# LessUp/n-body

Hardware: AMD Instinct MI355X
Metric: pair_interactions_per_s (higher is better)
Workload: dtype f32; 1 GPU; plummer_N1048576_direct_n2_velocity_verlet; bodies=1048576, seed=42, deterministic=True, deterministic_mode=1

## Files before the change

### n-body_amd/csrc/direct_sym.hip

```cpp

#include <type_traits>

#include "common.h"

namespace nbh {

typedef float f2 __attribute__((ext_vector_type(2)));

__device__ __forceinline__ float wave_rot1(float v) {
  return __int_as_float(__builtin_amdgcn_mov_dpp(__float_as_int(v), 0x134 , 0xF, 0xF, false));
}

constexpr int kSymBlocksPerCU = 16;
constexpr int kSymMinChunks = 4;
constexpr float kFar = 1.0e18f;

template <int R, bool RECT, bool EQM, bool DET = false>
__global__ __launch_bounds__(kBlock) void direct_sym_kernel(const float4* __restrict__ posm, int n,
                                                            const float4* __restrict__ posj, int nj,
                                                            int NB, int NBJ, int chunks_per_split,
                                                            double* __restrict__ acc64,
                                                            void* __restrict__ accj,
                                                            size_t plane_i, size_t plane_j,
                                                            const unsigned int* __restrict__ mass_range,
                                                            float eps2) {
  const bool uniform = mass_range[0] == mass_range[1] && mass_range[2] == mass_range[3] &&
                       mass_range[0] == mass_range[2] && ordered_to_float(mass_range[0]) > 0.f;
  if (uniform != EQM) return;
  const float m0 = EQM ? ordered_to_float(mass_range[0]) : 1.0f;
  constexpr int S = kBlock * R;
  __shared__ float slab[2][4][3][64];
  const int tid = threadIdx.x, lane = tid & 63, w = tid >> 6;
  const int A = blockIdx.x;
  const int D = RECT ? NBJ - 1 : NB / 2;
  constexpr int CPB = kBlock * R / 64;
  const int q0 = blockIdx.y * chunks_per_split;
  const int q1 = min((D + 1) * CPB, q0 + chunks_per_split);
  if (q0 >= q1) {
    if constexpr (DET) {
#pragma unroll
      for (int r = 0; r < R; r++)
#pragma unroll
        for (int c = 0; c < 3; c++)
          acc64[((size_t)blockIdx.y * 3 + c) * plane_i + (size_t)(A * S + r * kBlock + tid)] = 0.0;
    }
    return;
  }

  f2 xi[R / 2], yi[R / 2], zi[R / 2], mi[R / 2];
#pragma unroll
  for (int r = 0; r < R / 2; r++) {
    float4 p0 = make_float4(kFar, kFar, kFar, 0.f), p1 = p0;
    const int i0 = A * S + (2 * r) * kBlock + tid, i1 = i0 + kBlock;
    if (i0 < n) p0 = posm[i0];
    if (i1 < n) p1 = posm[i1];
    xi[r] = f2{p0.x, p1.x}; yi[r] = f2{p0.y, p1.y}; zi[r] = f2{p0.z, p1.z}; mi[r] = f2{p0.w, p1.w};
  }
  constexpr bool LACC = R >= 8;
  constexpr int RR = LACC ? 1 : R;
  __shared__ double lacc[LACC ? 3 * R * kBlock : 1];
  double sx[RR], sy[RR], sz[RR];
  if constexpr (LACC) {
#pragma unroll
    for (int k = 0; k < 3 * R; k++) lacc[k * kBlock + tid] = 0.0;
  } else {
#pragma unroll
    for (int r = 0; r < R; r++) sx[r] = sy[r] = sz[r] = 0.0;
  }
  f2 ax[R / 2], ay[R / 2], az[R / 2];
#pragma unroll
  for (int r = 0; r < R / 2; r++) ax[r] = ay[r] = az[r] = f2{0.f, 0.f};
  const f2 e2 = {eps2, eps2};

  auto partner_valid = [&](int d) { return RECT || !((NB % 2 == 0) && d == D && d > 0 && A >= D); };
  const int nchunks = q1 - q0;

  auto load_chunk = [&](int q) -> float4 {
    const int d = (q0 + q) / CPB, c = (q0 + q) % CPB;
    const int B = RECT ? d : (A + d) % NB;
    const int j = B * S + c * 64 + lane;
    float4 p = make_float4(kFar, kFar, kFar, 0.f);
    if (RECT) { if (j < nj) p = posj[j]; }
    else if (j < n && partner_valid(d)) p = posm[j];
    return p;
  };
  auto flush_chunk = [&](int q) {
    const int pd = (q0 + q) / CPB, pc = (q0 + q) % CPB;
    if constexpr (DET) {
      if (RECT || pd > 0) {
        const size_t plane = RECT ? plane_j : plane_i;
        float* slot = static_cast<float*>(accj) + (size_t)(RECT ? A : pd - 1) * 3 * plane;
        const unsigned int j = (unsigned int)((RECT ? pd : (A + pd) % NB) * S + pc * 64 + lane), pl = (unsigned int)plane;
        const int sb = q & 1;
        const bool keep = partner_valid(pd);
#pragma unroll
        for (int c = 0; c < 3; c++) {
          const float v = (slab[sb][0][c][lane] + slab[sb][1][c][lane]) + (slab[sb][2][c][lane] + slab[sb][3][c][lane]);
          slot[c * pl + j] = keep ? v : 0.f;
        }
      }
    } else if ((RECT || pd > 0) && partner_valid(pd)) {
      const int j = (RECT ? pd : (A + pd) % NB) * S + pc * 64 + lane;
      const int sb = q & 1;
      double* dst = RECT ? static_cast<double*>(accj) : acc64;
      const size_t plane = RECT ? plane_j : plane_i;
#pragma unroll
      for (int c = 0; c < 3; c++) {
        const float v = (slab[sb][0][c][lane] + slab[sb][1][c][lane]) + (slab[sb][2][c][lane] + slab[sb][3][c][lane]);
        unsafeAtomicAdd(&dst[c * plane + (size_t)j], (double)v * (double)m0);
      }
    }
  };

  float4 jnext = load_chunk(0);
  for (int q = 0; q < nchunks; q++) {
    const float4 jcur = jnext;
    if (q + 1 < nchunks) jnext = load_chunk(q + 1);
    const int d = (q0 + q) / CPB;
    const bool react = RECT || d > 0;
    if (q > 0) {
      __syncthreads();
      if (w == (q & 3)) flush_chunk(q - 1);
    }
    float jx = jcur.x, jy = jcur.y, jz = jcur.z, jm = jcur.w;
    float hjx = 0.f, hjy = 0.f, hjz = 0.f;
    auto steps = [&](auto react_tag) {
      constexpr bool REACT = decltype(react_tag)::value;
      constexpr int kStepUnroll = R >= 16 ? 1 : 2;
#pragma unroll kStepUnroll
      for (int k = 0; k < 64; k++) {
        const f2 sxj = {jx, jx}, syj = {jy, jy}, szj = {jz, jz}, smj = {jm, jm};
        f2 dx[R / 2], dy[R / 2], dz[R / 2], g[R / 2];
#pragma unroll
        for (int r = 0; r < R / 2; r++) {
          dx[r] = sxj - xi[r]; dy[r] = syj - yi[r]; dz[r] = szj - zi[r];
          g[r] = __builtin_elementwise_fma(dx[r], dx[r], __builtin_elementwise_fma(dy[r], dy[r], __builtin_elementwise_fma(dz[r], dz[r], e2)));
        }
#pragma unroll
        for (int r = 0; r < R / 2; r++) {
          g[r].x = __builtin_amdgcn_rsqf(g[r].x);
          g[r].y = __builtin_amdgcn_rsqf(g[r].y);
        }
#pragma unroll
        for (int r = 0; r < R / 2; r++) g[r] = (g[r] * g[r]) * g[r];
        f2 hx = {hjx, 0.f}, hy = {hjy, 0.f}, hz = {hjz, 0.f};
#pragma unroll
        for (int r = 0; r < R / 2; r++) {
          const f2 fj = EQM ? g[r] : g[r] * smj;
          ax[r] = __builtin_elementwise_fma(fj, dx[r], ax[r]);
          ay[r] = __builtin_elementwise_fma(fj, dy[r], ay[r]);
          az[r] = __builtin_elementwise_fma(fj, dz[r], az[r]);
          if (REACT) {
            const f2 fi = EQM ? g[r] : g[r] * mi[r];
            hx = __builtin_elementwise_fma(-fi, dx[r], hx);
            hy = __builtin_elementwise_fma(-fi, dy[r], hy);
            hz = __builtin_elementwise_fma(-fi, dz[r], hz);
          }
        }
        if (REACT) {
          hjx = wave_rot1(hx.x + hx.y); hjy = wave_rot1(hy.x + hy.y); hjz = wave_rot1(hz.x + hz.y);
        }
        jx = wave_rot1(jx); jy = wave_rot1(jy); jz = wave_rot1(jz); jm = wave_rot1(jm);
      }
    };
    if constexpr (R >= 12 && !EQM) {
      (void)react;
      steps(std::true_type{});
    } else {
      if (react) steps(std::true_type{}); else steps(std::false_type{});
    }
    slab[q & 1][w][0][lane] = hjx; slab[q & 1][w][1][lane] = hjy; slab[q & 1][w][2][lane] = hjz;
    if ((q & 3) == 3 || q == nchunks - 1) {
#pragma unroll
      for (int r = 0; r < R / 2; r++) {
        if constexpr (LACC) {
          lacc[(0 * R + 2 * r) * kBlock + tid] += (double)ax[r].x; lacc[(0 * R + 2 * r + 1) * kBlock + tid] += (double)ax[r].y;
          lacc[(1 * R + 2 * r) * kBlock + tid] += (double)ay[r].x; lacc[(1 * R + 2 * r + 1) * kBlock + tid] += (double)ay[r].y;
          lacc[(2 * R + 2 * r) * kBlock + tid] += (double)az[r].x; lacc[(2 * R + 2 * r + 1) * kBlock + tid] += (double)az[r].y;
        } else {
          sx[2 * r] += (double)ax[r].x; sx[2 * r + 1] += (double)ax[r].y;
          sy[2 * r] += (double)ay[r].x; sy[2 * r + 1] += (double)ay[r].y;
          sz[2 * r] += (double)az[r].x; sz[2 * r + 1] += (double)az[r].y;
        }
        ax[r] = ay[r] = az[r] = f2{0.f, 0.f};
      }
    }
  }
  __syncthreads();
  if (w == (nchunks & 3)) flush_chunk(nchunks - 1);
#pragma unroll
  for (int r = 0; r < R; r++) {
    const int i = A * S + r * kBlock + tid;
    const double fx = LACC ? lacc[(0 * R + r) * kBlock + tid] : sx[LACC ? 0 : r];
    const double fy = LACC ? lacc[(1 * R + r) * kBlock + tid] : sy[LACC ? 0 : r];
    const double fz = LACC ? lacc[(2 * R + r) * kBlock + tid] : sz[LACC ? 0 : r];
    if constexpr (DET) {
      double* slot = acc64 + (size_t)blockIdx.y * 3 * plane_i;
      const unsigned int iu = (unsigned int)i, pl = (unsigned int)plane_i;
      slot[iu] = fx;
      slot[pl + iu] = fy;
      slot[2u * pl + iu] = fz;
    } else {
      unsafeAtomicAdd(&acc64[(size_t)i], fx * (double)m0);
      unsafeAtomicAdd(&acc64[plane_i + (size_t)i], fy * (double)m0);
      unsafeAtomicAdd(&acc64[2 * plane_i + (size_t)i], fz * (double)m0);
    }
  }
}

__global__ void mass_range_init_kernel(unsigned int* enc) {
  if (threadIdx.x < 4) enc[threadIdx.x] = (threadIdx.x & 1) ? 0u : 0xffffffffu;
}

__global__ __launch_bounds__(kBlock) void mass_range_kernel(const float4* __restrict__ posm, int n,
                                                            unsigned int* __restrict__ enc) {
  __shared__ float red[4][2];
  float lo = INFINITY, hi = -INFINITY;
  for (int i = blockIdx.x * kBlock + threadIdx.x; i < n; i += gridDim.x * kBlock) {
    const float m = posm[i].w;
    lo = fminf(lo, m); hi = fmaxf(hi, m);
  }
#pragma unroll
  for (int off = 32; off > 0; off >>= 1) {
    lo = fminf(lo, __shfl_down(lo, off, 64));
    hi = fmaxf(hi, __shfl_down(hi, off, 64));
  }
  const int w = threadIdx.x >> 6;
  if ((threadIdx.x & 63) == 0) { red[w][0] = lo; red[w][1] = hi; }
  __syncthreads();
  if (threadIdx.x == 0) {
    for (int k = 1; k < 4; k++) { lo = fminf(lo, red[k][0]); hi = fmaxf(hi, red[k][1]); }
    atomicMin(&enc[0], float_to_ordered(fminf(lo, red[0][0])));
    atomicMax(&enc[1], float_to_ordered(fmaxf(hi, red[0][1])));
  }
}

struct SlotLayout {
  const double* isl;
  const float* rsl;
  size_t plane;
  int n_i, n_r;
};

__global__ __launch_bounds__(kBlock) void direct_sym_finalize_kernel(
    SlotLayout eq, SlotLayout gen, int apply_m0, const unsigned int* __restrict__ mass_range, int n, float G,
    float4* __restrict__ acc4, int accumulate, float* __restrict__ ax, float* __restrict__ ay, float* __restrict__ az,
    float* __restrict__ vx, float* __restrict__ vy, float* __restrict__ vz, const float* __restrict__ aox,
    const float* __restrict__ aoy, const float* __restrict__ aoz, float half_dt) {
  const int i = blockIdx.x * kBlock + threadIdx.x;
  if (i >= n) return;
  SlotLayout L = eq;
  double m0 = 1.0;
  if (mass_range) {
    const bool uniform = mass_range[0] == mass_range[1] && mass_range[2] == mass_range[3] &&
                         mass_range[0] == mass_range[2] && ordered_to_float(mass_range[0]) > 0.f;
    if (!uniform) L = gen;
    else if (apply_m0) m0 = (double)ordered_to_float(mass_range[0]);
  }
  double sx = 0.0, sy = 0.0, sz = 0.0;
  for (int k = 0; k < L.n_r; k++) {
    const float* p = L.rsl + (size_t)k * 3 * L.plane;
    sx += (double)p[i]; sy += (double)p[L.plane + i]; sz += (double)p[2 * L.plane + i];
  }
  for (int k = 0; k < L.n_i; k++) {
    const double* p = L.isl + (size_t)k * 3 * L.plane;
    sx += p[i]; sy += p[L.plane + i]; sz += p[2 * L.plane + i];
  }
  const double gm = (double)G * m0;
  const float fx = (float)(gm * sx), fy = (float)(gm * sy), fz = (float)(gm * sz);
  if (acc4) {
    float4 o = make_float4(fx, fy, fz, 0.f);
    if (accumulate) { const float4 c = acc4[i]; o.x += c.x; o.y += c.y; o.z += c.z; }
    acc4[i] = o;
  } else {
    ax[i] = fx; ay[i] = fy; az[i] = fz;
    if (vx) {
      vx[i] = kick1(vx[i], aox[i], fx, half_dt);
      vy[i] = kick1(vy[i], aoy[i], fy, half_dt);
      vz[i] = kick1(vz[i], aoz[i], fz, half_dt);
    }
  }
}

static void launch_mass_range(nbody_hip_ctx* ctx, const float4* pi, int ni, const float4* pj, int nj,
                              unsigned int* enc) {
  hipLaunchKernelGGL(mass_range_init_kernel, dim3(1), dim3(64), 0, ctx->stream, enc);
  const int bi = (ni + kBlock - 1) / kBlock, bj = (nj + kBlock - 1) / kBlock;
  hipLaunchKernelGGL(mass_range_kernel, dim3(bi < 256 ? bi : 256), dim3(kBlock), 0, ctx->stream, pi, ni, enc);
  hipLaunchKernelGGL(mass_range_kernel, dim3(bj < 256 ? bj : 256), dim3(kBlock), 0, ctx->stream, pj, nj, enc + 2);
}

template <int R, bool RECT, bool DET>
static void launch_sym(nbody_hip_ctx* ctx, dim3 grid, const float4* pi, int ni, const float4* pj, int nj,
                       int NB, int NBJ, int per, double* acci, void* accj, const unsigned int* enc,
                       float eps2) {
  const size_t S = (size_t)kBlock * R;
  hipLaunchKernelGGL((direct_sym_kernel<R, RECT, true, DET>), grid, dim3(kBlock), 0, ctx->stream, pi, ni, pj, nj,
                     NB, NBJ, per, acci, accj, (size_t)NB * S, (size_t)NBJ * S, enc, eps2);
  hipLaunchKernelGGL((direct_sym_kernel<R, RECT, false, DET>), grid, dim3(kBlock), 0, ctx->stream, pi, ni, pj, nj,
                     NB, NBJ, per, acci, accj, (size_t)NB * S, (size_t)NBJ * S, enc, eps2);
}

bool symmetric_pays(const nbody_hip_ctx* ctx, size_t n) {
  if (ctx->tune_variant == 3) return true;
  return ctx->tune_variant < 0 && n >= 12288;
}

static int sym_R(const nbody_hip_ctx* ctx, size_t n, bool two_sets) {
  if (ctx->tune_tpl == 2 || ctx->tune_tpl == 4 || ctx->tune_tpl == 6 || ctx->tune_tpl == 8 ||
      ctx->tune_tpl == 16 || (ctx->tune_tpl == 12 && !two_sets))
    return ctx->tune_tpl;
  if (two_sets) return n >= 49152 ? 16 : (n >= 16384 ? 8 : 4);
  return n >= 200000 ? 16 : (n >= 100000 ? 12 : (n >= 28000 ? 8 : 6));
}

static size_t align256(size_t b) { return (b + 255) & ~(size_t)255; }

SymShape sym_shape(const nbody_hip_ctx* ctx, size_t n, int R) {
  SymShape c;
  c.R = R;
  const int S = kBlock * R;
  c.NB = (int)((n + S - 1) / S);
  c.D = c.NB / 2;
  const int total = (c.D + 1) * (S / 64);
  int splits = ctx->tune_splits > 0 ? ctx->tune_splits : (kNumCU * kSymBlocksPerCU + c.NB - 1) / c.NB;
  if (splits < 1) splits = 1;
  int per = (total + splits - 1) / splits;
  if (per < kSymMinChunks) per = kSymMinChunks;
  if (per > S / 64) per = (per + S / 64 - 1) / (S / 64) * (S / 64);
  c.per = per;
  c.splits = (total + per - 1) / per;
  c.plane = (size_t)c.NB * S;
  return c;
}
size_t SymShape::reaction_bytes() const { return align256((size_t)D * 3 * plane * sizeof(float)); }
size_t SymShape::det_bytes() const { return reaction_bytes() + (size_t)splits * 3 * plane * sizeof(double); }
size_t SymShape::atomic_bytes() const { return 3 * plane * sizeof(double); }

static bool det_budget_allows(const nbody_hip_ctx* ctx, size_t bytes, size_t* free_now) {
  if (free_now) *free_now = 0;
  if (bytes > ctx->det_budget) return false;
  if (bytes <= ctx->partial.bytes) return true;
  size_t free_b = 0, total_b = 0;
  if (hipMemGetInfo(&free_b, &total_b) != hipSuccess) {
    (void)hipGetLastError();
    return true;
  }
  if (free_now) *free_now = free_b;
  return bytes <= (free_b + ctx->partial.bytes) / 4;
}

DirectPlan direct_plan(const nbody_hip_ctx* ctx, size_t n, bool query_device) {
  DirectPlan p;
  p.symmetric = symmetric_pays(ctx, n);
  p.eq = sym_shape(ctx, n, sym_R(ctx, n, false));
  p.gen = p.eq;
  p.det = false;
  p.bytes = 0;
  if (!p.symmetric) return p;
  if (ctx->deterministic) {
    SymShape gen = (kDetGenR != 16 && p.eq.R == 16 && ctx->tune_tpl == 0) ? sym_shape(ctx, n, kDetGenR) : p.eq;
    size_t need = p.eq.det_bytes() > gen.det_bytes() ? p.eq.det_bytes() : gen.det_bytes();
    bool ok = query_device ? det_budget_allows(ctx, need, nullptr) : need <= ctx->det_budget;
    if (!ok && gen.R != p.eq.R) {
      gen = p.eq;
      need = p.eq.det_bytes();
      ok = query_device ? det_budget_allows(ctx, need, nullptr) : need <= ctx->det_budget;
    }
    if (ok) {
      p.det = true;
      p.gen = gen;
      p.bytes = need;
    }
    p.det_bytes_wanted = need;
  }
  if (!p.det) p.bytes = p.eq.atomic_bytes();
  return p;
}

namespace {
template <int R, bool EQM, bool DET>
void launch_all_pairs(nbody_hip_ctx* ctx, const SymShape& c, const float4* posm, int n, double* acci, void* accj,
                      const unsigned int* enc, float eps2) {
  hipLaunchKernelGGL((direct_sym_kernel<R, false, EQM, DET>), dim3(c.NB, c.splits), dim3(kBlock), 0, ctx->stream, posm, n,
                     posm, n, c.NB, c.NB, c.per, acci, accj, c.plane, c.plane, enc, eps2);
}
template <bool EQM, bool DET>
void launch_all_pairs_R(nbody_hip_ctx* ctx, const SymShape& c, const float4* posm, int n, double* acci, void* accj,
                        const unsigned int* enc, float eps2) {
  switch (c.R) {
    case 2: launch_all_pairs<2, EQM, DET>(ctx, c, posm, n, acci, accj, enc, eps2); break;
    case 6: launch_all_pairs<6, EQM, DET>(ctx, c, posm, n, acci, accj, enc, eps2); break;
    case 8: launch_all_pairs<8, EQM, DET>(ctx, c, posm, n, acci, accj, enc, eps2); break;
    case 12: launch_all_pairs<12, EQM, DET>(ctx, c, posm, n, acci, accj, enc, eps2); break;
    case 16: launch_all_pairs<16, EQM, DET>(ctx, c, posm, n, acci, accj, enc, eps2); break;
    default: launch_all_pairs<4, EQM, DET>(ctx, c, posm, n, acci, accj, enc, eps2); break;
  }
}
}

int direct_symmetric(nbody_hip_ctx* ctx, const float4* posm, size_t n, float G, float eps2,
                     float4* acc4, int accumulate, float* ax, float* ay, float* az, float* vx,
                     float* vy, float* vz, const float* aox, const float* aoy, const float* aoz,
                     float half_dt) {
  DirectPlan plan = direct_plan(ctx, n, true);
  if (ctx->deterministic == 2 && !plan.det)
    return NBH_FAIL(NBODY_HIP_ERR_RESOURCE, "deterministic Direct sums were required but their slot planes (%zu bytes "
                    "for %zu bodies) exceed the budget (%zu bytes and a quarter of the free device memory)",
                    plan.det_bytes_wanted, n, ctx->det_budget);
  if (ctx->partial.bytes > ((size_t)64 << 20) && ctx->partial.bytes / 4 > plan.bytes && !ctx->capturing) {
    NBH_HIP(hipDeviceSynchronize());
    ctx->partial.release();
  }
  int rc = ctx->partial.reserve(plan.bytes);
  if (rc != NBODY_HIP_OK && plan.det && ctx->deterministic != 2) {
    (void)hipGetLastError();
    plan.det = false;
    plan.gen = plan.eq;
    plan.bytes = plan.eq.atomic_bytes();
    rc = ctx->partial.reserve(plan.bytes);
  }
  if (rc != NBODY_HIP_OK) return rc;
  const SymShape &eq = plan.eq, &gen = plan.gen;
  const bool det = plan.det;
  char* base = static_cast<char*>(ctx->partial.ptr);
  if (!det) NBH_HIP(hipMemsetAsync(base, 0, plan.bytes, ctx->stream));
  if (int rc2 = ctx->reduce.reserve(64)) return rc2;
  unsigned int* enc = static_cast<unsigned int*>(ctx->reduce.ptr);
  const int ni = (int)n;
  launch_mass_range(ctx, posm, ni, posm, ni, enc);
  SlotLayout Leq, Lgen;
  if (det) {
    Leq = SlotLayout{reinterpret_cast<const double*>(base + eq.reaction_bytes()), reinterpret_cast<const float*>(base),
                     eq.plane, eq.splits, eq.D};
    Lgen = SlotLayout{reinterpret_cast<const double*>(base + gen.reaction_bytes()), reinterpret_cast<const float*>(base),
                      gen.plane, gen.splits, gen.D};
    launch_all_pairs_R<true, true>(ctx, eq, posm, ni, const_cast<double*>(Leq.isl), base, enc, eps2);
    launch_all_pairs_R<false, true>(ctx, gen, posm, ni, const_cast<double*>(Lgen.isl), base, enc, eps2);
  } else {
    Leq = Lgen = SlotLayout{reinterpret_cast<const double*>(base), nullptr, eq.plane, 1, 0};
    launch_all_pairs_R<true, false>(ctx, eq, posm, ni, reinterpret_cast<double*>(base), base, enc, eps2);
    launch_all_pairs_R<false, false>(ctx, gen, posm, ni, reinterpret_cast<double*>(base), base, enc, eps2);
  }
  NBH_LAUNCH_CHECK();
  ctx->last_direct_kernel = det ? 2 : 1;
  const int fblocks = (int)((n + kBlock - 1) / kBlock);
  hipLaunchKernelGGL(direct_sym_finalize_kernel, dim3(fblocks), dim3(kBlock), 0, ctx->stream, Leq, Lgen, det ? 1 : 0, enc,
                     ni, G, acc4, accumulate, ax, ay, az, vx, vy, vz, aox, aoy, aoz, half_dt);
  NBH_LAUNCH_CHECK();
  return NBODY_HIP_OK;
}

int direct_symmetric_pair(nbody_hip_ctx* ctx, const float4* pi, size_t ni, const float4* pj, size_t nj,
                          float G, float eps2, float4* acc_i, int accumulate_i, float4* acc_j,
                          int accumulate_j) {
  int R = 0, NBI = 0, NBJ = 0, per = 0, splits = 0;
  size_t plane_i = 0, plane_j = 0, det_i = 0, det_j = 0;
  auto shape = [&](bool det_form) {
    const size_t nmin = ni < nj ? ni : nj;
    R = sym_R(ctx, nmin, true);
    if (det_form && ctx->tune_tpl == 0 && R > 8) R = 8;
    const int S = kBlock * R;
    NBI = (int)((ni + S - 1) / S);
    NBJ = (int)((nj + S - 1) / S);
    const int total = NBJ * (S / 64);
    const int per_cu = det_form ? kSymBlocksPerCU / 2 : kSymBlocksPerCU;
    splits = ctx->tune_splits > 0 ? ctx->tune_splits : (kNumCU * per_cu + NBI - 1) / NBI;
    if (splits < 1) splits = 1;
    per = (total + splits - 1) / splits;
    if (per < kSymMinChunks) per = kSymMinChunks;
    if (per > S / 64) per = (per + S / 64 - 1) / (S / 64) * (S / 64);
    splits = (total + per - 1) / per;
    plane_i = (size_t)NBI * S;
    plane_j = (size_t)NBJ * S;
    det_i = align256((size_t)splits * 3 * plane_i * sizeof(double));
    det_j = (size_t)NBI * 3 * plane_j * sizeof(float);
  };
  shape(ctx->deterministic != 0);
  bool det = ctx->deterministic != 0 && det_budget_allows(ctx, det_i + det_j, nullptr);
  if (ctx->deterministic == 2 && !det)
    return NBH_FAIL(NBODY_HIP_ERR_RESOURCE, "deterministic Direct sums were required but their slot planes (%zu bytes) "
                    "exceed the budget", det_i + det_j);
  if (!det) shape(false);
  size_t bi = align256(plane_i * 3 * sizeof(double)), bj = plane_j * 3 * sizeof(double);
  int rc = ctx->partial.reserve(det ? det_i + det_j : bi + bj);
  if (rc != NBODY_HIP_OK && det && ctx->deterministic != 2) {
    (void)hipGetLastError();
    det = false;
    shape(false);
    bi = align256(plane_i * 3 * sizeof(double));
    bj = plane_j * 3 * sizeof(double);
    rc = ctx->partial.reserve(bi + bj);
  }
  if (rc != NBODY_HIP_OK) return rc;
  char* base = static_cast<char*>(ctx->partial.ptr);
  double* acci = reinterpret_cast<double*>(base);
  void* accj = base + (det ? det_i : bi);
  if (!det) NBH_HIP(hipMemsetAsync(base, 0, bi + bj, ctx->stream));
  if (int rc2 = ctx->reduce.reserve(64)) return rc2;
  unsigned int* enc = static_cast<unsigned int*>(ctx->reduce.ptr);
  launch_mass_range(ctx, pi, (int)ni, pj, (int)nj, enc);
  const dim3 grid(NBI, splits);
#define NBH_PAIR_LAUNCH(RR)                                                                                          \
  if (det) launch_sym<RR, true, true>(ctx, grid, pi, (int)ni, pj, (int)nj, NBI, NBJ, per, acci, accj, enc, eps2);    \
  else launch_sym<RR, true, false>(ctx, grid, pi, (int)ni, pj, (int)nj, NBI, NBJ, per, acci, accj, enc, eps2)
  switch (R) {
    case 2: NBH_PAIR_LAUNCH(2); break;
    case 6: NBH_PAIR_LAUNCH(6); break;
    case 8: NBH_PAIR_LAUNCH(8); break;
    case 16: NBH_PAIR_LAUNCH(16); break;
    default: NBH_PAIR_LAUNCH(4); break;
  }
#undef NBH_PAIR_LAUNCH
  NBH_LAUNCH_CHECK();
  ctx->last_direct_kernel = det ? 2 : 1;
  SlotLayout Li, Lj;
  if (det) {
    Li = SlotLayout{acci, nullptr, plane_i, splits, 0};
    Lj = SlotLayout{nullptr, static_cast<const float*>(accj), plane_j, 0, NBI};
  } else {
    Li = SlotLayout{acci, nullptr, plane_i, 1, 0};
    Lj = SlotLayout{static_cast<const double*>(accj), nullptr, plane_j, 1, 0};
  }
  hipLaunchKernelGGL(direct_sym_finalize_kernel, dim3((unsigned)((ni + kBlock - 1) / kBlock)), dim3(kBlock), 0,
                     ctx->stream, Li, Li, det ? 1 : 0, det ? enc : nullptr, (int)ni, G, acc_i, accumulate_i, nullptr, nullptr,
                     nullptr, nullptr, nullptr, nullptr, nullptr, nullptr, nullptr, 0.f);
  hipLaunchKernelGGL(direct_sym_finalize_kernel, dim3((unsigned)((nj + kBlock - 1) / kBlock)), dim3(kBlock), 0,
                     ctx->stream, Lj, Lj, det ? 1 : 0, det ? enc : nullptr, (int)nj, G, acc_j, accumulate_j, nullptr, nullptr,
                     nullptr, nullptr, nullptr, nullptr, nullptr, nullptr, nullptr, 0.f);
  NBH_LAUNCH_CHECK();
  return NBODY_HIP_OK;
}

}
```

Before: 7033 billion pair-interactions/s.

## Batch reaction flushes per chunk group and split diagonal loop from react loop

```diff
diff --git a/n-body_amd/csrc/direct_sym.hip b/n-body_amd/csrc/direct_sym.hip
--- a/n-body_amd/csrc/direct_sym.hip
+++ b/n-body_amd/csrc/direct_sym.hip
@@ -29,8 +29,10 @@
   if (uniform != EQM) return;
   const float m0 = EQM ? ordered_to_float(mass_range[0]) : 1.0f;
   constexpr int S = kBlock * R;
-  __shared__ float slab[2][4][3][64];
-  const int tid = threadIdx.x, lane = tid & 63, w = tid >> 6;
+  constexpr int G = R == 12 ? 1 : (R == 2 ? 2 : 4);
+  __shared__ float slab[2][G][4][3][64];
+  const int tid = threadIdx.x, lane = tid & 63;
+  const int w = __builtin_amdgcn_readfirstlane(tid >> 6);
   const int A = blockIdx.x;
   const int D = RECT ? NBJ - 1 : NB / 2;
   constexpr int CPB = kBlock * R / 64;
@@ -73,121 +75,132 @@
   const f2 e2 = {eps2, eps2};
 
   auto partner_valid = [&](int d) { return RECT || !((NB % 2 == 0) && d == D && d > 0 && A >= D); };
+  auto partner = [&](int d) { return A + d >= NB ? A + d - NB : A + d; };
   const int nchunks = q1 - q0;
 
   auto load_chunk = [&](int q) -> float4 {
     const int d = (q0 + q) / CPB, c = (q0 + q) % CPB;
-    const int B = RECT ? d : (A + d) % NB;
+    const int B = RECT ? d : partner(d);
     const int j = B * S + c * 64 + lane;
     float4 p = make_float4(kFar, kFar, kFar, 0.f);
     if (RECT) { if (j < nj) p = posj[j]; }
     else if (j < n && partner_valid(d)) p = posm[j];
     return p;
   };
-  auto flush_chunk = [&](int q) {
+  auto flush_chunk = [&](int q, const float (*sums)[3][64]) {
     const int pd = (q0 + q) / CPB, pc = (q0 + q) % CPB;
     if constexpr (DET) {
       if (RECT || pd > 0) {
         const size_t plane = RECT ? plane_j : plane_i;
         float* slot = static_cast<float*>(accj) + (size_t)(RECT ? A : pd - 1) * 3 * plane;
-        const unsigned int j = (unsigned int)((RECT ? pd : (A + pd) % NB) * S + pc * 64 + lane), pl = (unsigned int)plane;
-        const int sb = q & 1;
+        const unsigned int j = (unsigned int)((RECT ? pd : partner(pd)) * S + pc * 64 + lane), pl = (unsigned int)plane;
         const bool keep = partner_valid(pd);
 #pragma unroll
         for (int c = 0; c < 3; c++) {
-          const float v = (slab[sb][0][c][lane] + slab[sb][1][c][lane]) + (slab[sb][2][c][lane] + slab[sb][3][c][lane]);
+          const float v = (sums[0][c][lane] + sums[1][c][lane]) + (sums[2][c][lane] + sums[3][c][lane]);
           slot[c * pl + j] = keep ? v : 0.f;
         }
       }
     } else if ((RECT || pd > 0) && partner_valid(pd)) {
-      const int j = (RECT ? pd : (A + pd) % NB) * S + pc * 64 + lane;
-      const int sb = q & 1;
+      const int j = (RECT ? pd : partner(pd)) * S + pc * 64 + lane;
       double* dst = RECT ? static_cast<double*>(accj) : acc64;
       const size_t plane = RECT ? plane_j : plane_i;
 #pragma unroll
       for (int c = 0; c < 3; c++) {
-        const float v = (slab[sb][0][c][lane] + slab[sb][1][c][lane]) + (slab[sb][2][c][lane] + slab[sb][3][c][lane]);
+        const float v = (sums[0][c][lane] + sums[1][c][lane]) + (sums[2][c][lane] + sums[3][c][lane]);
         unsafeAtomicAdd(&dst[c * plane + (size_t)j], (double)v * (double)m0);
       }
     }
   };
 
+  auto flush_group = [&](int g, int count) {
+    const int k = (w - g - 1) & 3;
+    if (k < count) flush_chunk(g * G + k, slab[g & 1][k]);
+  };
+
   float4 jnext = load_chunk(0);
-  for (int q = 0; q < nchunks; q++) {
+  auto chunk = [&](int q, auto react_tag) {
+    constexpr bool REACT = decltype(react_tag)::value;
     const float4 jcur = jnext;
     if (q + 1 < nchunks) jnext = load_chunk(q + 1);
-    const int d = (q0 + q) / CPB;
-    const bool react = RECT || d > 0;
-    if (q > 0) {
+    const int grp = q / G, k = q % G;
+    if (k == 0 && q > 0) {
       __syncthreads();
-      if (w == (q & 3)) flush_chunk(q - 1);
+      flush_group(grp - 1, G);
     }
     float jx = jcur.x, jy = jcur.y, jz = jcur.z, jm = jcur.w;
     float hjx = 0.f, hjy = 0.f, hjz = 0.f;
-    auto steps = [&](auto react_tag) {
-      constexpr bool REACT = decltype(react_tag)::value;
-      constexpr int kStepUnroll = R >= 16 ? 1 : 2;
+    constexpr int kStepUnroll = R >= 16 ? 1 : 2;
 #pragma unroll kStepUnroll
-      for (int k = 0; k < 64; k++) {
-        const f2 sxj = {jx, jx}, syj = {jy, jy}, szj = {jz, jz}, smj = {jm, jm};
-        f2 dx[R / 2], dy[R / 2], dz[R / 2], g[R / 2];
+    for (int s = 0; s < 64; s++) {
+      const f2 sxj = {jx, jx}, syj = {jy, jy}, szj = {jz, jz}, smj = {jm, jm};
+      f2 dx[R / 2], dy[R / 2], dz[R / 2], g[R / 2];
+#pragma unroll
+      for (int r = 0; r < R / 2; r++) {
+        dx[r] = sxj - xi[r]; dy[r] = syj - yi[r]; dz[r] = szj - zi[r];
+        g[r] = __builtin_elementwise_fma(dx[r], dx[r], __builtin_elementwise_fma(dy[r], dy[r], __builtin_elementwise_fma(dz[r], dz[r], e2)));
+      }
+#pragma unroll
+      for (int r = 0; r < R / 2; r++) {
+        g[r].x = __builtin_amdgcn_rsqf(g[r].x);
+        g[r].y = __builtin_amdgcn_rsqf(g[r].y);
+      }
+#pragma unroll
+      for (int r = 0; r < R / 2; r++) g[r] = (g[r] * g[r]) * g[r];
+      f2 hx = {hjx, 0.f}, hy = {hjy, 0.f}, hz = {hjz, 0.f};
+#pragma unroll
+      for (int r = 0; r < R / 2; r++) {
+        const f2 fj = EQM ? g[r] : g[r] * smj;
+        ax[r] = __builtin_elementwise_fma(fj, dx[r], ax[r]);
+        ay[r] = __builtin_elementwise_fma(fj, dy[r], ay[r]);
+        az[r] = __builtin_elementwise_fma(fj, dz[r], az[r]);
+        if (REACT) {
+          const f2 fi = EQM ? g[r] : g[r] * mi[r];
+          hx = __builtin_elementwise_fma(-fi, dx[r], hx);
+          hy = __builtin_elementwise_fma(-fi, dy[r], hy);
+          hz = __builtin_elementwise_fma(-fi, dz[r], hz);
+        }
+      }
+      if (REACT) {
+        hjx = wave_rot1(hx.x + hx.y); hjy = wave_rot1(hy.x + hy.y); hjz = wave_rot1(hz.x + hz.y);
+      }
+      jx = wave_rot1(jx); jy = wave_rot1(jy); jz = wave_rot1(jz); jm = wave_rot1(jm);
+    }
+    slab[grp & 1][k][w][0][lane] = hjx; slab[grp & 1][k][w][1][lane] = hjy; slab[grp & 1][k][w][2][lane] = hjz;
+    if ((q & 3) == 3 || q == nchunks - 1) {
+      if constexpr (LACC) {
+        auto fold = [&](int comp, f2 (&a)[R / 2]) {
+          double t[R];
+#pragma unroll
+          for (int r = 0; r < R; r++) t[r] = lacc[(comp * R + r) * kBlock + tid];
+#pragma unroll
+          for (int r = 0; r < R / 2; r++) {
+            t[2 * r] += (double)a[r].x; t[2 * r + 1] += (double)a[r].y;
+            a[r] = f2{0.f, 0.f};
+          }
+#pragma unroll
+          for (int r = 0; r < R; r++) lacc[(comp * R + r) * kBlock + tid] = t[r];
+        };
+        fold(0, ax); fold(1, ay); fold(2, az);
+      } else {
 #pragma unroll
         for (int r = 0; r < R / 2; r++) {
-          dx[r] = sxj - xi[r]; dy[r] = syj - yi[r]; dz[r] = szj - zi[r];
-          g[r] = __builtin_elementwise_fma(dx[r], dx[r], __builtin_elementwise_fma(dy[r], dy[r], __builtin_elementwise_fma(dz[r], dz[r], e2)));
-        }
-#pragma unroll
-        for (int r = 0; r < R / 2; r++) {
-          g[r].x = __builtin_amdgcn_rsqf(g[r].x);
-          g[r].y = __builtin_amdgcn_rsqf(g[r].y);
-        }
-#pragma unroll
-        for (int r = 0; r < R / 2; r++) g[r] = (g[r] * g[r]) * g[r];
-        f2 hx = {hjx, 0.f}, hy = {hjy, 0.f}, hz = {hjz, 0.f};
-#pragma unroll
-        for (int r = 0; r < R / 2; r++) {
-          const f2 fj = EQM ? g[r] : g[r] * smj;
-          ax[r] = __builtin_elementwise_fma(fj, dx[r], ax[r]);
-          ay[r] = __builtin_elementwise_fma(fj, dy[r], ay[r]);
-          az[r] = __builtin_elementwise_fma(fj, dz[r], az[r]);
-          if (REACT) {
-            const f2 fi = EQM ? g[r] : g[r] * mi[r];
-            hx = __builtin_elementwise_fma(-fi, dx[r], hx);
-            hy = __builtin_elementwise_fma(-fi, dy[r], hy);
-            hz = __builtin_elementwise_fma(-fi, dz[r], hz);
-          }
-        }
-        if (REACT) {
-          hjx = wave_rot1(hx.x + hx.y); hjy = wave_rot1(hy.x + hy.y); hjz = wave_rot1(hz.x + hz.y);
-        }
-        jx = wave_rot1(jx); jy = wave_rot1(jy); jz = wave_rot1(jz); jm = wave_rot1(jm);
-      }
-    };
-    if constexpr (R >= 12 && !EQM) {
-      (void)react;
-      steps(std::true_type{});
-    } else {
-      if (react) steps(std::true_type{}); else steps(std::false_type{});
-    }
-    slab[q & 1][w][0][lane] = hjx; slab[q & 1][w][1][lane] = hjy; slab[q & 1][w][2][lane] = hjz;
-    if ((q & 3) == 3 || q == nchunks - 1) {
-#pragma unroll
-      for (int r = 0; r < R / 2; r++) {
-        if constexpr (LACC) {
-          lacc[(0 * R + 2 * r) * kBlock + tid] += (double)ax[r].x; lacc[(0 * R + 2 * r + 1) * kBlock + tid] += (double)ax[r].y;
-          lacc[(1 * R + 2 * r) * kBlock + tid] += (double)ay[r].x; lacc[(1 * R + 2 * r + 1) * kBlock + tid] += (double)ay[r].y;
-          lacc[(2 * R + 2 * r) * kBlock + tid] += (double)az[r].x; lacc[(2 * R + 2 * r + 1) * kBlock + tid] += (double)az[r].y;
-        } else {
           sx[2 * r] += (double)ax[r].x; sx[2 * r + 1] += (double)ax[r].y;
           sy[2 * r] += (double)ay[r].x; sy[2 * r + 1] += (double)ay[r].y;
           sz[2 * r] += (double)az[r].x; sz[2 * r + 1] += (double)az[r].y;
+          ax[r] = ay[r] = az[r] = f2{0.f, 0.f};
         }
-        ax[r] = ay[r] = az[r] = f2{0.f, 0.f};
-      }
-    }
-  }
+      }
+    }
+  };
+  int q = 0;
+  if constexpr (!RECT && !(R >= 12 && !EQM)) {
+    const int ndiag = min(nchunks, max(0, CPB - q0));
+    for (; q < ndiag; q++) chunk(q, std::false_type{});
+  }
+  for (; q < nchunks; q++) chunk(q, std::true_type{});
   __syncthreads();
-  if (w == (nchunks & 3)) flush_chunk(nchunks - 1);
+  flush_group((nchunks - 1) / G, nchunks - (nchunks - 1) / G * G);
 #pragma unroll
   for (int r = 0; r < R; r++) {
     const int i = A * S + r * kBlock + tid;
```

After: 7078 billion pair-interactions/s, median of 6. About the same (+0.6%).

## Track chunk position incrementally, split flush across waves, and peel self-block loop

Applied to the files above, without the earlier changes.

```diff
diff --git a/n-body_amd/csrc/direct_sym.hip b/n-body_amd/csrc/direct_sym.hip
--- a/n-body_amd/csrc/direct_sym.hip
+++ b/n-body_amd/csrc/direct_sym.hip
@@ -75,57 +75,68 @@
   auto partner_valid = [&](int d) { return RECT || !((NB % 2 == 0) && d == D && d > 0 && A >= D); };
   const int nchunks = q1 - q0;
 
-  auto load_chunk = [&](int q) -> float4 {
-    const int d = (q0 + q) / CPB, c = (q0 + q) % CPB;
-    const int B = RECT ? d : (A + d) % NB;
-    const int j = B * S + c * 64 + lane;
-    float4 p = make_float4(kFar, kFar, kFar, 0.f);
-    if (RECT) { if (j < nj) p = posj[j]; }
-    else if (j < n && partner_valid(d)) p = posm[j];
-    return p;
-  };
-  auto flush_chunk = [&](int q) {
-    const int pd = (q0 + q) / CPB, pc = (q0 + q) % CPB;
+  struct ChunkPos {
+    int d, c;
+    int j0;
+    int counts;
+    size_t slot;
+  };
+  auto set_partner = [&](ChunkPos& p, int d) {
+    p.d = d;
+    p.c = 0;
+    p.j0 = (RECT ? d : (A + d) % NB) * S;
+    p.counts = partner_valid(d);
+    p.slot = (size_t)(RECT ? A : (d > 0 ? d - 1 : 0)) * 3 * (RECT ? plane_j : plane_i);
+  };
+  auto advance = [&](ChunkPos& p) {
+    if (++p.c == CPB) set_partner(p, p.d + 1);
+    else p.j0 += 64;
+  };
+  const float4* __restrict__ jsrc = RECT ? posj : posm;
+  const int jlast = (RECT ? nj : n) - 1;
+  auto load_chunk = [&](const ChunkPos& p) -> float4 { return jsrc[min(p.j0 + lane, jlast)]; };
+  auto flush_chunk = [&](const ChunkPos& p, int q) {
+    if (w == 3) return;
+    const int sb = q & 1;
+    const unsigned int j = (unsigned int)(p.j0 + lane);
+    auto sum4 = [&](int c) { return (slab[sb][0][c][lane] + slab[sb][1][c][lane]) + (slab[sb][2][c][lane] + slab[sb][3][c][lane]); };
     if constexpr (DET) {
-      if (RECT || pd > 0) {
-        const size_t plane = RECT ? plane_j : plane_i;
-        float* slot = static_cast<float*>(accj) + (size_t)(RECT ? A : pd - 1) * 3 * plane;
-        const unsigned int j = (unsigned int)((RECT ? pd : (A + pd) % NB) * S + pc * 64 + lane), pl = (unsigned int)plane;
-        const int sb = q & 1;
-        const bool keep = partner_valid(pd);
-#pragma unroll
-        for (int c = 0; c < 3; c++) {
-          const float v = (slab[sb][0][c][lane] + slab[sb][1][c][lane]) + (slab[sb][2][c][lane] + slab[sb][3][c][lane]);
-          slot[c * pl + j] = keep ? v : 0.f;
-        }
+      if (RECT || p.d > 0) {
+        float* slot = static_cast<float*>(accj) + p.slot;
+        const unsigned int pl = (unsigned int)(RECT ? plane_j : plane_i);
+        const float v = sum4(w);
+        slot[(unsigned int)w * pl + j] = p.counts ? v : 0.f;
       }
-    } else if ((RECT || pd > 0) && partner_valid(pd)) {
-      const int j = (RECT ? pd : (A + pd) % NB) * S + pc * 64 + lane;
-      const int sb = q & 1;
+    } else if ((RECT || p.d > 0) && p.counts) {
       double* dst = RECT ? static_cast<double*>(accj) : acc64;
       const size_t plane = RECT ? plane_j : plane_i;
-#pragma unroll
-      for (int c = 0; c < 3; c++) {
-        const float v = (slab[sb][0][c][lane] + slab[sb][1][c][lane]) + (slab[sb][2][c][lane] + slab[sb][3][c][lane]);
-        unsafeAtomicAdd(&dst[c * plane + (size_t)j], (double)v * (double)m0);
-      }
-    }
-  };
-
-  float4 jnext = load_chunk(0);
-  for (int q = 0; q < nchunks; q++) {
-    const float4 jcur = jnext;
-    if (q + 1 < nchunks) jnext = load_chunk(q + 1);
-    const int d = (q0 + q) / CPB;
-    const bool react = RECT || d > 0;
+      unsafeAtomicAdd(&dst[(size_t)w * plane + (size_t)j], (double)sum4(w) * (double)m0);
+    }
+  };
+
+  auto select_chunk = [&](const float4& raw, const ChunkPos& p) -> float4 {
+    const bool ok = p.counts && p.j0 + lane <= jlast;
+    return make_float4(ok ? raw.x : kFar, ok ? raw.y : kFar, ok ? raw.z : kFar, ok ? raw.w : 0.f);
+  };
+  ChunkPos cur;
+  set_partner(cur, q0 / CPB);
+  cur.c = q0 % CPB;
+  cur.j0 += cur.c * 64;
+  ChunkPos prv = cur, nxt = cur;
+  float4 jraw = load_chunk(cur);
+  float4 jsel = select_chunk(jraw, cur);
+  auto chunk = [&](int q, auto react_tag) {
+    float jx = jsel.x, jy = jsel.y, jz = jsel.z, jm = jsel.w;
+    nxt = cur;
+    advance(nxt);
+    jraw = load_chunk(nxt);
     if (q > 0) {
       __syncthreads();
-      if (w == (q & 3)) flush_chunk(q - 1);
-    }
-    float jx = jcur.x, jy = jcur.y, jz = jcur.z, jm = jcur.w;
+      flush_chunk(prv, q - 1);
+    }
     float hjx = 0.f, hjy = 0.f, hjz = 0.f;
-    auto steps = [&](auto react_tag) {
-      constexpr bool REACT = decltype(react_tag)::value;
+    auto steps = [&](auto tag) {
+      constexpr bool REACT = decltype(tag)::value;
       constexpr int kStepUnroll = R >= 16 ? 1 : 2;
 #pragma unroll kStepUnroll
       for (int k = 0; k < 64; k++) {
@@ -164,10 +175,10 @@
       }
     };
     if constexpr (R >= 12 && !EQM) {
-      (void)react;
+      (void)react_tag;
       steps(std::true_type{});
     } else {
-      if (react) steps(std::true_type{}); else steps(std::false_type{});
+      steps(react_tag);
     }
     slab[q & 1][w][0][lane] = hjx; slab[q & 1][w][1][lane] = hjy; slab[q & 1][w][2][lane] = hjz;
     if ((q & 3) == 3 || q == nchunks - 1) {
@@ -185,9 +196,18 @@
         ax[r] = ay[r] = az[r] = f2{0.f, 0.f};
       }
     }
+    jsel = select_chunk(jraw, nxt);
+    prv = cur;
+    cur = nxt;
+  };
+  {
+    int q = 0;
+    if constexpr (!RECT && !(R >= 12 && !EQM))
+      for (; q < nchunks && cur.d == 0; q++) chunk(q, std::false_type{});
+    for (; q < nchunks; q++) chunk(q, std::true_type{});
   }
   __syncthreads();
-  if (w == (nchunks & 3)) flush_chunk(nchunks - 1);
+  flush_chunk(prv, nchunks - 1);
 #pragma unroll
   for (int r = 0; r < R; r++) {
     const int i = A * S + r * kBlock + tid;
```

After: 6707 billion pair-interactions/s before, 6761 billion pair-interactions/s after, median of 6. Within noise of the previous version (+0.8%).
